# fabsig/GPBoost

Hardware: NVIDIA H100
Metric: gp_loglik_evals_per_sec (higher is better)
Workload: dtype f64

## Files before the change

### gpboost_b200/csrc/dev/dev_api.cu

```cuda
#include "../../../include/gpboost_b200_dev.h"

#include <cuda_runtime.h>

#include <algorithm>
#include <cmath>
#include <numeric>
#include <cstdio>
#include <cstring>
#include <string>
#include <vector>

#include "knn.cuh"
#include "vecchia_factor.cuh"
#include "vecchia_big.cuh"
#include "vecchia_nll2.cuh"

namespace {

thread_local std::string g_last_error;

int fail(const std::string& msg) {
  g_last_error = msg;
  return -1;
}

#define CUDA_TRY(expr)                                                                              \
  do {                                                                                              \
    cudaError_t err__ = (expr);                                                                     \
    if (err__ != cudaSuccess) {                                                                     \
      return fail(std::string("CUDA error at " __FILE__ ":") + std::to_string(__LINE__) + ": " +    \
                  cudaGetErrorString(err__));                                                       \
    }                                                                                               \
  } while (0)


__global__ void gather_perm_kernel(const double* __restrict__ src, const int32_t* __restrict__ perm,
                                   double* __restrict__ dst, int64_t n) {
  for (int64_t i = (int64_t)blockIdx.x * blockDim.x + threadIdx.x; i < n; i += (int64_t)gridDim.x * blockDim.x)
    dst[i] = src[perm[i]];
}

__global__ void reduce_partials_kernel(const double* __restrict__ partials, int64_t nrows, double* __restrict__ out) {
  __shared__ double sh[256];
  for (int k = 0; k < gpb::kNumAcc; ++k) {
    double s = 0.;
    for (int64_t r = threadIdx.x; r < nrows; r += blockDim.x) s += partials[r * gpb::kNumAcc + k];
    sh[threadIdx.x] = s;
    __syncthreads();
    for (int o = blockDim.x / 2; o > 0; o >>= 1) {
      if (threadIdx.x < o) sh[threadIdx.x] += sh[threadIdx.x + o];
      __syncthreads();
    }
    if (threadIdx.x == 0) out[k] = sh[0];
    __syncthreads();
  }
}

__global__ void bt_apply_kernel(const double* __restrict__ A, const double* __restrict__ u,
                                const int32_t* __restrict__ colptr, const int32_t* __restrict__ csc_pos,
                                const int32_t* __restrict__ perm, double* __restrict__ out_orig, int64_t n, int m,
                                int64_t row_begin, int64_t row_end, double scale) {
  const int lane = threadIdx.x & 31;
  const int64_t warp = ((int64_t)blockIdx.x * blockDim.x + threadIdx.x) >> 5;
  const int64_t nwarps = ((int64_t)gridDim.x * blockDim.x) >> 5;
  for (int64_t j = warp; j < n; j += nwarps) {
    const int32_t b = colptr[j], e = colptr[j + 1];
    double s = 0.;
    for (int32_t p = b + lane; p < e; p += 32) {
      const int32_t pos = csc_pos[p];
      s -= A[pos] * u[pos / m];
    }
    s = gpb::warp_sum(s);
    if (lane == 0) {
      if (j >= row_begin && j < row_end) s += u[j];
      out_orig[perm[j]] = s * scale;
    }
  }
}

__global__ void fill_kernel(double* p, int64_t n, double v) {
  for (int64_t i = (int64_t)blockIdx.x * blockDim.x + threadIdx.x; i < n; i += (int64_t)gridDim.x * blockDim.x) p[i] = v;
}

__global__ void fp64_peak_kernel(double* out, int iters, double a, double b) {
  double x0 = threadIdx.x, x1 = x0 + 1., x2 = x0 + 2., x3 = x0 + 3., x4 = x0 + 4., x5 = x0 + 5., x6 = x0 + 6., x7 = x0 + 7.;
  for (int i = 0; i < iters; ++i) {
    x0 = fma(x0, a, b); x1 = fma(x1, a, b); x2 = fma(x2, a, b); x3 = fma(x3, a, b);
    x4 = fma(x4, a, b); x5 = fma(x5, a, b); x6 = fma(x6, a, b); x7 = fma(x7, a, b);
  }
  if (x0 + x1 + x2 + x3 + x4 + x5 + x6 + x7 == 12345.678) out[0] = x0;
}

using FactorKernel = void (*)(const gpb::FactorArgs);

template <int COV, int MODE, int DIM>
FactorKernel pick_cap(int m) {
  if (m <= 10) return gpb::vecchia_factor_kernel<COV, MODE, DIM, 10>;
  if (m <= 20) return gpb::vecchia_factor_kernel<COV, MODE, DIM, 20>;
// ... 124 lines not shown
      const int32_t j = h->nn_host[(size_t)i * m + k];
      if (j >= 0) ++colptr[j + 1];
    }
  for (int64_t j = 0; j < n; ++j) colptr[j + 1] += colptr[j];
  std::vector<int32_t> pos((size_t)colptr[n]);
  std::vector<int32_t> fill(colptr.begin(), colptr.end() - 1);
  for (int64_t i = h->row_begin; i < h->row_end; ++i)
    for (int k = 0; k < m; ++k) {
      const int32_t j = h->nn_host[(size_t)i * m + k];
      if (j >= 0) pos[fill[j]++] = (int32_t)(i * m + k);
    }
  CUDA_TRY(cudaMalloc(&h->colptr, sizeof(int32_t) * (n + 1)));
  CUDA_TRY(cudaMalloc(&h->csc_pos, sizeof(int32_t) * std::max<size_t>(pos.size(), 1)));
  CUDA_TRY(cudaMemcpy(h->colptr, colptr.data(), sizeof(int32_t) * (n + 1), cudaMemcpyHostToDevice));
  CUDA_TRY(cudaMemcpy(h->csc_pos, pos.data(), sizeof(int32_t) * pos.size(), cudaMemcpyHostToDevice));
  CUDA_TRY(cudaMalloc(&h->yaux, sizeof(double) * n));
  return 0;
}

int launch_eval(gpbdev_vecchia* h, int cov_type, double var, double range, int mode, bool latent = false) {
  if (cov_type < 0 || cov_type > 3) return fail("gpbdev_vecchia_eval: unknown covariance id");
  if (mode < 0 || mode > 3) return fail("gpbdev_vecchia_eval: unknown mode");
  if (!(var > 0.) || !(range > 0.)) return fail("gpbdev_vecchia_eval: covariance parameters must be positive");
  CUDA_TRY(cudaSetDevice(h->device));
  if (mode == gpb::MODE_STORE && !latent && h->factor_stored && h->stored_cov == cov_type && h->stored_latent == latent &&
      h->stored_var == var && h->stored_range == range && h->last_cov == cov_type && h->last_latent == latent && h->last_var == var &&
      h->last_range == range)
    return 0;
  if (mode == gpb::MODE_STORE || mode == gpb::MODE_STORE_GRAD) {
    if (ensure_store_buffers(h)) return -1;
  }
  h->last_cov = cov_type; h->last_latent = latent; h->last_var = var; h->last_range = range;
  if (mode == gpb::MODE_STORE || mode == gpb::MODE_STORE_GRAD) { h->stored_cov = cov_type; h->stored_latent = latent; h->stored_var = var; h->stored_range = range; }
  if (mode == gpb::MODE_STORE_GRAD && !h->dA) {
    CUDA_TRY(cudaMalloc(&h->dA, sizeof(double) * h->n * h->m));
    CUDA_TRY(cudaMalloc(&h->dD, sizeof(double) * h->n));
    CUDA_TRY(cudaMemsetAsync(h->dA, 0, sizeof(double) * h->n * h->m, h->stream));
    CUDA_TRY(cudaMemsetAsync(h->dD, 0, sizeof(double) * h->n, h->stream));
  }
  gpb::FactorArgs a;
  a.coords = h->coords; a.nn = h->nn; a.y = h->y;
  a.A = h->A; a.Dinv = h->Dinv; a.w = h->u;
  a.partials = h->partials;
  a.n = h->n; a.row_begin = h->row_begin; a.row_end = h->row_end;
  a.m = h->m; a.d = h->d; a.var = var; a.range = range;
  a.diag_nb = latent ? var * (1. + 1e-10) : var + 1.;
  a.diag_obs = latent ? var : var + 1.;
  if (mode == gpb::MODE_STORE_GRAD) {
    CUDA_TRY(cudaMemcpyToSymbolAsync(gpb::g_factor_dA, &h->dA, sizeof(double*), 0, cudaMemcpyHostToDevice, h->stream));
    CUDA_TRY(cudaMemcpyToSymbolAsync(gpb::g_factor_dD, &h->dD, sizeof(double*), 0, cudaMemcpyHostToDevice, h->stream));
  }
  if (latent && mode == gpb::MODE_GRAD) return fail("gpbdev_vecchia_eval: the gradient pass assumes a Gaussian likelihood");
  auto finish = [&](int64_t rows) -> int {
    CUDA_TRY(cudaGetLastError());
    reduce_partials_kernel<<<1, 256, 0, h->stream>>>(h->partials, rows, h->sums);
    CUDA_TRY(cudaGetLastError());
    h->launches += 2;
    if (h->allreduce && !latent) {
      if (h->allreduce(h->allreduce_ctx, h->sums, gpb::kNumAcc, (void*)h->stream)) return fail("gpbdev_vecchia_eval: device all-reduce failed");
    }
    if (mode == gpb::MODE_STORE || mode == gpb::MODE_STORE_GRAD) h->factor_stored = true;
    return 0;
  };
  if (h->m > gpb::kMaxNeighbors) {
    if (mode == gpb::MODE_STORE_GRAD) return fail("gpbdev_vecchia_eval: the factor derivative (non-Gaussian likelihoods) supports num_neighbors <= 30");
    gpb::BigArgs b;
    b.coords = h->coords; b.y = h->y; b.nn = h->nn; b.qcoords = nullptr;
    b.A = h->A; b.Dinv = h->Dinv; b.w = h->u; b.pred_mean = nullptr; b.pred_var = nullptr; b.partials = h->partials;
    b.row_begin = h->row_begin; b.row_end = h->row_end; b.m = h->m; b.d = h->d;
    b.var = var; b.range = range; b.diag_nb = a.diag_nb; b.diag_obs = a.diag_obs;
    const int bmode = mode == gpb::MODE_NLL ? gpb::BIG_NLL : (mode == gpb::MODE_STORE ? gpb::BIG_STORE : gpb::BIG_GRAD);
    const int warps = bmode == gpb::BIG_GRAD ? 2 : 4;
    BigKernel bk = pick_big_kernel(cov_type, bmode);
    const size_t bsmem = gpb::big_smem_bytes(bmode, warps, h->d);
    CUDA_TRY(cudaFuncSetAttribute(bk, cudaFuncAttributeMaxDynamicSharedMemorySize, (int)bsmem));
    int grid = std::min(h->num_sms, (int)((h->grid_cap * gpb::kWarpsPerBlock) / warps));
    grid = std::max(grid, 1);
    bk<<<grid, warps * 32, bsmem, h->stream>>>(b);
    return finish((int64_t)grid * warps);
  }
  if ((mode == gpb::MODE_NLL || mode == gpb::MODE_STORE || (mode == gpb::MODE_GRAD && !latent)) && h->d == 2 && h->m > 20) {
    FactorKernel k2 = nullptr;
#define GPB_PICK2(COVID)                                                                                                              \
    k2 = mode == gpb::MODE_NLL ? gpb::vecchia_nll2_kernel<COVID, gpb::MODE_NLL>                                                      \
         : (mode == gpb::MODE_STORE ? gpb::vecchia_nll2_kernel<COVID, gpb::MODE_STORE> : gpb::vecchia_nll2_kernel<COVID, gpb::MODE_GRAD>)
    switch (cov_type) {
      case gpb::COV_EXPONENTIAL: GPB_PICK2(gpb::COV_EXPONENTIAL); break;
      case gpb::COV_MATERN15: GPB_PICK2(gpb::COV_MATERN15); break;
      case gpb::COV_MATERN25: GPB_PICK2(gpb::COV_MATERN25); break;
      default: GPB_PICK2(gpb::COV_GAUSSIAN); break;
    }
#undef GPB_PICK2
    const size_t smem2 = sizeof(double) * gpb::kWarpsPerBlock * 2 * (gpb::kNll2Half + 64);
    CUDA_TRY(cudaFuncSetAttribute(k2, cudaFuncAttributeMaxDynamicSharedMemorySize, (int)smem2));
    CUDA_TRY(cudaFuncSetAttribute(k2, cudaFuncAttributePreferredSharedMemoryCarveout, cudaSharedmemCarveoutMaxShared));
    int per_sm2 = 0;
    CUDA_TRY(cudaOccupancyMaxActiveBlocksPerMultiprocessor(&per_sm2, k2, gpb::kWarpsPerBlock * 32, smem2));
    int grid2 = std::max(per_sm2, 1) * h->num_sms;
    grid2 = std::max(1, std::min(grid2, h->grid_cap / 2));
    k2<<<grid2, gpb::kWarpsPerBlock * 32, smem2, h->stream>>>(a);
    if (finish((int64_t)grid2 * gpb::kWarpsPerBlock * 2)) return -1;
    if (mode == gpb::MODE_GRAD && a.A != nullptr) {
      h->factor_stored = true;
      h->stored_cov = cov_type; h->stored_latent = false; h->stored_var = var; h->stored_range = range;
    }
    return 0;
  }
  FactorKernel k = pick_kernel(cov_type, mode, h->d, h->m);
  if (!k) return fail("gpbdev_vecchia_eval: no one-observation factor kernel for this mode at d = 2, num_neighbors > 20");
  const size_t smem = sizeof(double) * gpb::kWarpsPerBlock * (32 * gpb::kLd + 32 * h->d + 64);
  CUDA_TRY(cudaFuncSetAttribute(k, cudaFuncAttributeMaxDynamicSharedMemorySize, (int)smem));
  CUDA_TRY(cudaFuncSetAttribute(k, cudaFuncAttributePreferredSharedMemoryCarveout, cudaSharedmemCarveoutMaxShared));
  int per_sm = 0;
  CUDA_TRY(cudaOccupancyMaxActiveBlocksPerMultiprocessor(&per_sm, k, gpb::kWarpsPerBlock * 32, smem));
  int grid = std::max(per_sm, 1) * h->num_sms;
  if (grid > h->grid_cap) grid = h->grid_cap;
  k<<<grid, gpb::kWarpsPerBlock * 32, smem, h->stream>>>(a);
  return finish((int64_t)grid * gpb::kWarpsPerBlock);
}

}

extern "C" {

const char* gpbdev_last_error(void) { return g_last_error.c_str(); }

int gpbdev_vecchia_set_allreduce(gpbdev_vecchia_t h, gpbdev_allreduce_fn fn, void* ctx) {
  if (!h) return fail("gpbdev_vecchia_set_allreduce: null argument");
  h->allreduce = fn;
  h->allreduce_ctx = ctx;
  return 0;
}

int gpbdev_device_count(void) {
  int c = 0;
  if (cudaGetDeviceCount(&c) != cudaSuccess) { cudaGetLastError(); return 0; }
  return c;
}

int gpbdev_vecchia_create(gpbdev_vecchia_t* out, int device, int64_t n, int d, int m, const double* coords_ordered,
                          const int32_t* perm, const int32_t* nn, int64_t row_begin, int64_t row_end) {
  if (!out || !coords_ordered || !perm) return fail("gpbdev_vecchia_create: null argument");
  if (n <= 0 || d <= 0 || d > 16) return fail("gpbdev_vecchia_create: need n > 0 and 1 <= dim <= 16");
  if (m < 1 || m > gpb::kBigMaxNeighbors)
    return fail("gpbdev_vecchia_create: num_neighbors must be in [1, " + std::to_string(gpb::kBigMaxNeighbors) +
                "] for the CUDA Vecchia engine");
  if ((int64_t)n * m >= (int64_t)2147483647) return fail("gpbdev_vecchia_create: n * num_neighbors exceeds int32 positions");
  if (row_begin < 0 || row_end > n || row_begin > row_end) return fail("gpbdev_vecchia_create: bad row shard");
  if (nn) {
    std::vector<int64_t> seen((size_t)n, -1);
    for (int64_t i = 0; i < n; ++i)
      for (int k = 0; k < m; ++k) {
        const int32_t j = nn[i * m + k];
        if (j == -1) continue;
        if (j < -1 || j >= i)
          return fail("gpbdev_vecchia_create: neighbour " + std::to_string(j) + " of row " + std::to_string(i) +
                      " is neither -1 nor an earlier row");
        if (seen[(size_t)j] == i)
          return fail("gpbdev_vecchia_create: neighbour " + std::to_string(j) + " appears twice in row " + std::to_string(i));
        seen[(size_t)j] = i;
      }
  }
  if (gpbdev_device_count() <= device)
    return fail("gpbdev_vecchia_create: no CUDA device " + std::to_string(device) + " — the CUDA engine has no CPU fallback");
  CUDA_TRY(cudaSetDevice(device));
  gpbdev_vecchia* h = new gpbdev_vecchia();
  h->device = device; h->n = n; h->d = d; h->m = m; h->row_begin = row_begin; h->row_end = row_end;
  cudaDeviceProp prop;
  CUDA_TRY(cudaGetDeviceProperties(&prop, device));
  h->num_sms = prop.multiProcessorCount;
  CUDA_TRY(cudaStreamCreateWithFlags(&h->stream, cudaStreamNonBlocking));
  CUDA_TRY(cudaEventCreate(&h->ev0));
  CUDA_TRY(cudaEventCreate(&h->ev1));
  CUDA_TRY(cudaMalloc(&h->coords, sizeof(double) * n * d));
  CUDA_TRY(cudaMalloc(&h->nn, sizeof(int32_t) * n * m));
  CUDA_TRY(cudaMalloc(&h->perm, sizeof(int32_t) * n));
// ... 263 lines not shown
  CUDA_TRY(cudaStreamSynchronize(h->stream));
  CUDA_TRY(cudaMemcpy(A_host, h->A, sizeof(double) * h->n * h->m, cudaMemcpyDeviceToHost));
  CUDA_TRY(cudaMemcpy(Dinv_host, h->Dinv, sizeof(double) * h->n, cudaMemcpyDeviceToHost));
  CUDA_TRY(cudaMemcpy(dA_host, h->dA, sizeof(double) * h->n * h->m, cudaMemcpyDeviceToHost));
  CUDA_TRY(cudaMemcpy(dD_host, h->dD, sizeof(double) * h->n, cudaMemcpyDeviceToHost));
  return 0;
}

int gpbdev_vecchia_get_factor(gpbdev_vecchia_t h, double* A_host, double* Dinv_host) {
  if (!h || !A_host || !Dinv_host) return fail("gpbdev_vecchia_get_factor: null argument");
  if (!h->factor_stored) return fail("gpbdev_vecchia_get_factor: call gpbdev_vecchia_eval(mode=STORE) first");
  CUDA_TRY(cudaSetDevice(h->device));
  CUDA_TRY(cudaStreamSynchronize(h->stream));
  CUDA_TRY(cudaMemcpy(A_host, h->A, sizeof(double) * h->n * h->m, cudaMemcpyDeviceToHost));
  CUDA_TRY(cudaMemcpy(Dinv_host, h->Dinv, sizeof(double) * h->n, cudaMemcpyDeviceToHost));
  return 0;
}

int gpbdev_vecchia_timer_start(gpbdev_vecchia_t h) {
  if (!h) return fail("null handle");
  CUDA_TRY(cudaSetDevice(h->device));
  CUDA_TRY(cudaEventRecord(h->ev0, h->stream));
  return 0;
}
int gpbdev_vecchia_timer_stop(gpbdev_vecchia_t h, float* ms) {
  if (!h || !ms) return fail("null argument");
  CUDA_TRY(cudaSetDevice(h->device));
  CUDA_TRY(cudaEventRecord(h->ev1, h->stream));
  CUDA_TRY(cudaEventSynchronize(h->ev1));
  CUDA_TRY(cudaEventElapsedTime(ms, h->ev0, h->ev1));
  return 0;
}
int gpbdev_vecchia_sync(gpbdev_vecchia_t h) {
  if (!h) return fail("null handle");
  CUDA_TRY(cudaSetDevice(h->device));
  CUDA_TRY(cudaStreamSynchronize(h->stream));
  return 0;
}
int64_t gpbdev_vecchia_launch_count(gpbdev_vecchia_t h) { return h ? h->launches : 0; }
int gpbdev_vecchia_knn_replayed(gpbdev_vecchia_t h) { return h ? h->knn_replayed : 0; }

int gpbdev_knn_search(int device, const double* coords_host, int64_t n, int d, int m, int64_t q_begin, int64_t end_search_at,
                      int32_t* nn_host, int64_t* info_out) {
  if (!coords_host || !nn_host || !info_out) return fail("gpbdev_knn_search: null argument");
  if (d < 1) return fail("gpbdev_knn_search: need dim >= 1");
  if (m < 1 || m > gpb::kBigMaxNeighbors)
    return fail("gpbdev_knn_search: num_neighbors must be in [1, " + std::to_string(gpb::kBigMaxNeighbors) + "]");
  if (n < 1 || n >= (int64_t)2147483647) return fail("gpbdev_knn_search: need 1 <= n < 2^31");
  if (q_begin < 0 || q_begin >= n) return fail("gpbdev_knn_search: q_begin must be in [0, n)");
  if (end_search_at != (q_begin == 0 ? n - 2 : q_begin - 1))
    return fail("gpbdev_knn_search: end_search_at must be n - 2 for model queries (q_begin = 0) and q_begin - 1 for prediction");
  m = (int)std::min<int64_t>(m, end_search_at + 1);
  if (m < 1) return fail("gpbdev_knn_search: model queries need n >= 2");
  const int64_t nq = n - q_begin;
  if (nq * m >= (int64_t)2147483647) return fail("gpbdev_knn_search: n * num_neighbors exceeds int32 positions");
  if (gpbdev_device_count() <= device) return fail("gpbdev_knn_search: no CUDA device " + std::to_string(device));
  CUDA_TRY(cudaSetDevice(device));
  cudaDeviceProp prop;
  CUDA_TRY(cudaGetDeviceProperties(&prop, device));
  cudaStream_t stream = nullptr;
  double* coords_dev = nullptr;
  int32_t* nn_dev = nullptr;
  CUDA_TRY(cudaStreamCreateWithFlags(&stream, cudaStreamNonBlocking));
  auto release = [&]() { cudaFree(coords_dev); cudaFree(nn_dev); cudaStreamDestroy(stream); };
  cudaError_t e = cudaMalloc(&coords_dev, sizeof(double) * n * d);
  if (e == cudaSuccess) e = cudaMalloc(&nn_dev, sizeof(int32_t) * nq * m);
  if (e == cudaSuccess) e = cudaMemcpy(coords_dev, coords_host, sizeof(double) * n * d, cudaMemcpyHostToDevice);
  if (e != cudaSuccess) { release(); return fail(std::string("gpbdev_knn_search: ") + cudaGetErrorString(e)); }
  std::string err;
  gpb::KnnInfo info;
  if (gpb::knn_vecchia_search(coords_dev, coords_host, n, d, m, nn_dev, stream, prop.multiProcessorCount, &info, &err, q_begin,
                              end_search_at) < 0) {
    release();
    return fail("gpbdev_knn_search: " + err);
  }
  e = cudaMemcpy(nn_host, nn_dev, sizeof(int32_t) * nq * m, cudaMemcpyDeviceToHost);
  release();
  if (e != cudaSuccess) return fail(std::string("gpbdev_knn_search: ") + cudaGetErrorString(e));
  const int64_t vals[7] = {info.replayed, info.launches, info.brute_end, info.ncell, info.g[0], info.g[1], info.g[2]};
  std::memcpy(info_out, vals, sizeof(vals));
  return 0;
}

int gpbdev_fp64_peak(int device, double* tflops) {
  if (!tflops) return fail("null argument");
  CUDA_TRY(cudaSetDevice(device));
  cudaDeviceProp prop;
  CUDA_TRY(cudaGetDeviceProperties(&prop, device));
  double* out = nullptr;
  CUDA_TRY(cudaMalloc(&out, 8));
  cudaEvent_t e0, e1;
  CUDA_TRY(cudaEventCreate(&e0));
  CUDA_TRY(cudaEventCreate(&e1));
  const int blocks = prop.multiProcessorCount * 8, threads = 256, iters = 1 << 14;
  fp64_peak_kernel<<<blocks, threads>>>(out, 1 << 10, 1.0000001, 1e-9);
  double best = 0.;
  for (int rep = 0; rep < 5; ++rep) {
    CUDA_TRY(cudaEventRecord(e0));
    fp64_peak_kernel<<<blocks, threads>>>(out, iters, 1.0000001, 1e-9);
    CUDA_TRY(cudaEventRecord(e1));
    CUDA_TRY(cudaEventSynchronize(e1));
    float ms = 0.f;
    CUDA_TRY(cudaEventElapsedTime(&ms, e0, e1));
    const double flops = 2.0 * 8 * (double)iters * blocks * threads;
    best = std::max(best, flops / (ms * 1e-3) / 1e12);
  }
  cudaEventDestroy(e0); cudaEventDestroy(e1); cudaFree(out);
  *tflops = best;
  return 0;
}

int gpbdev_vecchia_flush_l2(gpbdev_vecchia_t h) {
  if (!h) return fail("null handle");
  CUDA_TRY(cudaSetDevice(h->device));
  if (!h->flush) {
    h->flush_n = (int64_t)(256 << 20) / sizeof(double);
    CUDA_TRY(cudaMalloc(&h->flush, sizeof(double) * h->flush_n));
  }
  fill_kernel<<<h->num_sms * 8, 256, 0, h->stream>>>(h->flush, h->flush_n, 1.0);
  CUDA_TRY(cudaGetLastError());
  return 0;
}

}

#include "newton.cuh"
#include "covariates.cuh"
#include "laplace.cuh"
#include "fisher.cuh"
```

### include/gpboost_b200_dev.h

```cpp
#ifndef GPBOOST_B200_DEV_H_
#define GPBOOST_B200_DEV_H_
#include <stdint.h>
#ifdef __cplusplus
extern "C" {
#endif

#define GPBDEV_EXPORT __attribute__((visibility("default")))

enum { GPBDEV_COV_EXPONENTIAL = 0, GPBDEV_COV_MATERN15 = 1, GPBDEV_COV_MATERN25 = 2, GPBDEV_COV_GAUSSIAN = 3 };
enum { GPBDEV_MODE_NLL = 0, GPBDEV_MODE_STORE = 1, GPBDEV_MODE_GRAD = 2 };
enum {
  GPBDEV_SUM_QUAD = 0,
  GPBDEV_SUM_LOGDET = 1,
  GPBDEV_SUM_NBAD = 2,
  GPBDEV_SUM_UKU0 = 3, GPBDEV_SUM_UKU1 = 4,
  GPBDEV_SUM_UDU0 = 5, GPBDEV_SUM_UDU1 = 6,
  GPBDEV_SUM_TR0 = 7, GPBDEV_SUM_TR1 = 8,
  GPBDEV_NUM_SUMS = 9
};

typedef struct gpbdev_vecchia* gpbdev_vecchia_t;

GPBDEV_EXPORT const char* gpbdev_last_error(void);
GPBDEV_EXPORT int gpbdev_device_count(void);

GPBDEV_EXPORT int gpbdev_vecchia_create(gpbdev_vecchia_t* out, int device, int64_t n, int d, int m,
                                        const double* coords_ordered, const int32_t* perm,
                                        const int32_t* nn, int64_t row_begin, int64_t row_end);
GPBDEV_EXPORT int gpbdev_vecchia_free(gpbdev_vecchia_t h);

GPBDEV_EXPORT int gpbdev_vecchia_get_nn(gpbdev_vecchia_t h, int32_t* nn_host);

GPBDEV_EXPORT int gpbdev_vecchia_set_y(gpbdev_vecchia_t h, const double* y_host);
GPBDEV_EXPORT int gpbdev_vecchia_set_y_device(gpbdev_vecchia_t h, const double* y_dev);

GPBDEV_EXPORT int gpbdev_vecchia_eval(gpbdev_vecchia_t h, int cov_type, double var, double range, int mode,
                                      double* out);
GPBDEV_EXPORT int gpbdev_vecchia_eval_async(gpbdev_vecchia_t h, int cov_type, double var, double range, int mode);
GPBDEV_EXPORT int gpbdev_vecchia_last_sums(gpbdev_vecchia_t h, double* out);

GPBDEV_EXPORT int gpbdev_vecchia_yaux(gpbdev_vecchia_t h, double* yaux_host);
GPBDEV_EXPORT int gpbdev_vecchia_yaux_device(gpbdev_vecchia_t h, double* out_dev, double scale);
GPBDEV_EXPORT int gpbdev_vecchia_laplace_time_ops(gpbdev_vecchia_t h, int t, int reps, float* out_ms);
GPBDEV_EXPORT int gpbdev_vecchia_predict(gpbdev_vecchia_t h, int cov_type, double var, double range, const double* coords_pred_host,
                                         int64_t np, int num_neighbors_pred, double* mean_out_host, double* var_out_host);
typedef struct gpbdev_vecchia_predset* gpbdev_vecchia_predset_t;
GPBDEV_EXPORT int gpbdev_vecchia_predset_create(gpbdev_vecchia_t h, const double* coords_pred_host, int64_t np, int num_neighbors_pred,
                                                gpbdev_vecchia_predset_t* out);
GPBDEV_EXPORT int gpbdev_vecchia_predset_eval(gpbdev_vecchia_predset_t ps, int cov_type, double var, double range, const double** mean_dev,
                                              const double** var_dev);
GPBDEV_EXPORT int gpbdev_vecchia_predset_free(gpbdev_vecchia_predset_t ps);
GPBDEV_EXPORT int gpbdev_vecchia_newton_system(gpbdev_vecchia_t h, const int32_t* leaf_of_row_dev, int num_leaves, const double* grad_dev,
                                               double* M_host, double* rhs_host);
GPBDEV_EXPORT int gpbdev_vecchia_set_covariates(gpbdev_vecchia_t h, const double* X_colmajor_host, int p);
GPBDEV_EXPORT int gpbdev_vecchia_gls_gram(gpbdev_vecchia_t h, double* G_host, double* r_host);
GPBDEV_EXPORT int gpbdev_vecchia_gls_residual(gpbdev_vecchia_t h, const double* beta_host, double* out3);
GPBDEV_EXPORT int gpbdev_vecchia_latent_factor_grad(gpbdev_vecchia_t h, int cov_type, double var, double range, double* A_host,
                                                    double* Dinv_host, double* dA_host, double* dD_host);
GPBDEV_EXPORT int gpbdev_vecchia_fisher_info(gpbdev_vecchia_t h, int cov_type, double sigma2, double var, double range,
                                             const double* probes_colmajor, int t, double* FI9);
GPBDEV_EXPORT int gpbdev_vecchia_get_factor(gpbdev_vecchia_t h, double* A_host, double* Dinv_host);

GPBDEV_EXPORT int gpbdev_vecchia_timer_start(gpbdev_vecchia_t h);
GPBDEV_EXPORT int gpbdev_vecchia_timer_stop(gpbdev_vecchia_t h, float* ms);
GPBDEV_EXPORT int gpbdev_vecchia_sync(gpbdev_vecchia_t h);
GPBDEV_EXPORT int64_t gpbdev_vecchia_launch_count(gpbdev_vecchia_t h);
GPBDEV_EXPORT int gpbdev_vecchia_knn_replayed(gpbdev_vecchia_t h);
GPBDEV_EXPORT int gpbdev_knn_search(int device, const double* coords_host, int64_t n, int d, int m, int64_t q_begin,
                                    int64_t end_search_at, int32_t* nn_host, int64_t* info_out);
typedef int (*gpbdev_allreduce_fn)(void* ctx, double* dev_buf, int64_t count, void* stream);
GPBDEV_EXPORT int gpbdev_vecchia_set_allreduce(gpbdev_vecchia_t h, gpbdev_allreduce_fn fn, void* ctx);
GPBDEV_EXPORT int gpbdev_fp64_peak(int device, double* tflops);
GPBDEV_EXPORT int gpbdev_vecchia_flush_l2(gpbdev_vecchia_t h);

enum { GPBDEV_LIK_BERNOULLI_LOGIT = 0, GPBDEV_LIK_POISSON = 1 };
GPBDEV_EXPORT int gpbdev_vecchia_laplace_set_likelihood(gpbdev_vecchia_t h, int likelihood, double log_norm_const);
GPBDEV_EXPORT int gpbdev_laplace_rows(int device, int likelihood, int64_t n, const double* y_host, const double* mode_host,
                                      const double* fe_host, const double* Dinv_host, double* out_host);
GPBDEV_EXPORT int gpbdev_vecchia_laplace_set_probes(gpbdev_vecchia_t h, const double* probes_colmajor, int t);
GPBDEV_EXPORT int gpbdev_vecchia_laplace_eval(gpbdev_vecchia_t h, int cov_type, double var, double range,
                                              const double* fixed_effects_host, const double* cfg, double* out);
GPBDEV_EXPORT int gpbdev_vecchia_laplace_get_mode(gpbdev_vecchia_t h, double* mode_host);
GPBDEV_EXPORT int gpbdev_vecchia_laplace_keep_solutions(gpbdev_vecchia_t h, int keep);
GPBDEV_EXPORT int gpbdev_vecchia_laplace_grad(gpbdev_vecchia_t h, int cov_type, double var, double range, const double* cfg, double* out);
GPBDEV_EXPORT int gpbdev_vecchia_laplace_set_collective(gpbdev_vecchia_t h, void (*allreduce_sum)(double*, int), int t_total);
GPBDEV_EXPORT int gpbdev_vecchia_laplace_apply(gpbdev_vecchia_t h, int cov_type, double var, double range, int op, int t,
                                               const double* W_host, const double* X_host, const double* X2_host, double* out_host,
                                               double* dots_host);

typedef struct gpbdev_dense* gpbdev_dense_t;
GPBDEV_EXPORT const char* gpbdev_dense_last_error(void);
GPBDEV_EXPORT int gpbdev_dense_create(gpbdev_dense_t* out, int device, int n, int d, const double* coords_rowmajor);
GPBDEV_EXPORT int gpbdev_dense_free(gpbdev_dense_t h);
GPBDEV_EXPORT int gpbdev_dense_set_y(gpbdev_dense_t h, const double* y_host);
GPBDEV_EXPORT int gpbdev_dense_eval(gpbdev_dense_t h, int cov_type, double var, double range, double* out3);
GPBDEV_EXPORT int gpbdev_dense_yaux(gpbdev_dense_t h, double scale, double* yaux_host);
GPBDEV_EXPORT int gpbdev_dense_grad(gpbdev_dense_t h, double* out4);
GPBDEV_EXPORT int gpbdev_dense_get_factor(gpbdev_dense_t h, double* L_host, double* z_host);
GPBDEV_EXPORT int gpbdev_dense_get_psi_inv(gpbdev_dense_t h, double* P_host);
GPBDEV_EXPORT int64_t gpbdev_dense_launch_count(gpbdev_dense_t h);

typedef struct gpbdev_grouped* gpbdev_grouped_t;
GPBDEV_EXPORT const char* gpbdev_grouped_last_error(void);
GPBDEV_EXPORT int gpbdev_grouped_create(gpbdev_grouped_t* out, int device, int64_t n, const int32_t* group_index, int num_groups);
GPBDEV_EXPORT int gpbdev_grouped_free(gpbdev_grouped_t h);
GPBDEV_EXPORT int gpbdev_grouped_set_y(gpbdev_grouped_t h, const double* y_host);
GPBDEV_EXPORT int gpbdev_grouped_eval(gpbdev_grouped_t h, double var_ratio, double* out5);
GPBDEV_EXPORT int gpbdev_grouped_yaux(gpbdev_grouped_t h, double var_ratio, double scale, double* yaux_host);
GPBDEV_EXPORT int gpbdev_grouped_set_y_device(gpbdev_grouped_t h, const double* y_dev);
GPBDEV_EXPORT int gpbdev_grouped_yaux_device(gpbdev_grouped_t h, double var_ratio, double scale, double* out_dev);
GPBDEV_EXPORT int64_t gpbdev_grouped_launch_count(gpbdev_grouped_t h);

typedef struct gpbdev_grouped_multi* gpbdev_grouped_multi_t;
GPBDEV_EXPORT int gpbdev_grouped_multi_create(gpbdev_grouped_multi_t* out, int device, int64_t n, int K, const int32_t* level_index,
                                              const int* num_levels);
GPBDEV_EXPORT int gpbdev_grouped_multi_free(gpbdev_grouped_multi_t h);
GPBDEV_EXPORT int gpbdev_grouped_multi_info(gpbdev_grouped_multi_t h, int64_t* out2);
GPBDEV_EXPORT int gpbdev_grouped_multi_set_y(gpbdev_grouped_multi_t h, const double* y_host);
GPBDEV_EXPORT int gpbdev_grouped_multi_set_y_device(gpbdev_grouped_multi_t h, const double* y_dev);
GPBDEV_EXPORT int gpbdev_grouped_multi_set_probes(gpbdev_grouped_multi_t h, const double* probes, int t);
GPBDEV_EXPORT int gpbdev_grouped_multi_eval(gpbdev_grouped_multi_t h, const double* v, const double* cfg, double* out5);
GPBDEV_EXPORT int gpbdev_grouped_multi_grad(gpbdev_grouped_multi_t h, double sigma2, double* grad);
GPBDEV_EXPORT int gpbdev_grouped_multi_yaux(gpbdev_grouped_multi_t h, const double* v, const double* cfg, double scale, double* out,
                                            int out_is_device, int* its);
GPBDEV_EXPORT int gpbdev_grouped_multi_apply(gpbdev_grouped_multi_t h, const double* v, int which, const double* X, int t, double* Y);
GPBDEV_EXPORT int gpbdev_grouped_multi_time_ops(gpbdev_grouped_multi_t h, int reps, float* out_ms);
GPBDEV_EXPORT int64_t gpbdev_grouped_multi_launch_count(gpbdev_grouped_multi_t h);

typedef struct gpbdev_tree* gpbdev_tree_t;
typedef struct {
  int num_leaves;
  int min_data_in_leaf;
  double min_sum_hessian_in_leaf;
  double lambda_l2;
  double min_gain_to_split;
  int max_depth;
} gpbdev_tree_config;

GPBDEV_EXPORT const char* gpbdev_tree_last_error(void);
GPBDEV_EXPORT int gpbdev_tree_create(gpbdev_tree_t* out, int device, int64_t n, int F, const uint8_t* bins_feature_major,
                                     const int32_t* num_bin, const gpbdev_tree_config* cfg);
GPBDEV_EXPORT int gpbdev_tree_create_on_device_bins(gpbdev_tree_t* out, int device, int64_t n, int F, int Fpad, const uint8_t* bins_dev,
                                                    const int32_t* num_bin, const gpbdev_tree_config* cfg);
GPBDEV_EXPORT int gpbdev_tree_free(gpbdev_tree_t h);

GPBDEV_EXPORT const char* gpbdev_bin_last_error(void);
GPBDEV_EXPORT int gpbdev_bin_matrix(int device, const void* data_host, int data_type, int64_t nrow, int ncol, int is_row_major, int F,
                                    const int32_t* real_feature, const int32_t* num_bin, const double* upper_bounds,
                                    int upper_bounds_stride, int Fpad, uint8_t** bins_dev_out);
GPBDEV_EXPORT int gpbdev_bin_free(int device, uint8_t* bins_dev);
GPBDEV_EXPORT int gpbdev_bin_download(int device, const uint8_t* bins_dev, int64_t nrow, int Fpad, uint8_t* out_host);
GPBDEV_EXPORT int gpbdev_tree_train(gpbdev_tree_t h, const double* grad, int grad_on_device, double hess_const, int* num_leaves,
                                    int* split_feature, int* threshold_bin, int* left_child, int* right_child, float* split_gain,
                                    double* leaf_value, int* leaf_count);
GPBDEV_EXPORT int gpbdev_tree_add_score(gpbdev_tree_t h, const double* leaf_values, int num_leaves, double* score_dev,
// ... 41 lines not shown
```

Baseline: 323.8.

## Add FP64 tensor-core blocked Cholesky kernel for Vecchia NLL evaluation

After: 346.3, median of 6. 1.07x the previous value.

```diff
diff --git a/gpboost_b200/csrc/dev/dev_api.cu b/gpboost_b200/csrc/dev/dev_api.cu
--- a/gpboost_b200/csrc/dev/dev_api.cu
+++ b/gpboost_b200/csrc/dev/dev_api.cu
@@ -14,6 +14,7 @@
 #include "vecchia_factor.cuh"
 #include "vecchia_big.cuh"
 #include "vecchia_nll2.cuh"
+#include "vecchia_nll_mma.cuh"
 
 namespace {
 
@@ -304,7 +305,7 @@
   if ((mode == gpb::MODE_NLL || mode == gpb::MODE_STORE || (mode == gpb::MODE_GRAD && !latent)) && h->d == 2 && h->m > 20) {
     FactorKernel k2 = nullptr;
 #define GPB_PICK2(COVID)                                                                                                              \
-    k2 = mode == gpb::MODE_NLL ? gpb::vecchia_nll2_kernel<COVID, gpb::MODE_NLL>                                                      \
+    k2 = mode == gpb::MODE_NLL ? gpb::vecchia_nll_mma_kernel<COVID>                                                                  \
          : (mode == gpb::MODE_STORE ? gpb::vecchia_nll2_kernel<COVID, gpb::MODE_STORE> : gpb::vecchia_nll2_kernel<COVID, gpb::MODE_GRAD>)
     switch (cov_type) {
       case gpb::COV_EXPONENTIAL: GPB_PICK2(gpb::COV_EXPONENTIAL); break;
@@ -313,7 +314,8 @@
       default: GPB_PICK2(gpb::COV_GAUSSIAN); break;
     }
 #undef GPB_PICK2
-    const size_t smem2 = sizeof(double) * gpb::kWarpsPerBlock * 2 * (gpb::kNll2Half + 64);
+    const size_t smem2 = mode == gpb::MODE_NLL ? gpb::kWarpsPerBlock * gpb::kMmaSmemPerWarp
+                                               : sizeof(double) * gpb::kWarpsPerBlock * 2 * (gpb::kNll2Half + 64);
     CUDA_TRY(cudaFuncSetAttribute(k2, cudaFuncAttributeMaxDynamicSharedMemorySize, (int)smem2));
     CUDA_TRY(cudaFuncSetAttribute(k2, cudaFuncAttributePreferredSharedMemoryCarveout, cudaSharedmemCarveoutMaxShared));
     int per_sm2 = 0;
@@ -743,6 +745,20 @@
   return 0;
 }
 
+int gpbdev_dmma_m8n8k4(const double* a, const double* b, const double* c, double* d) {
+  if (!a || !b || !c || !d) return fail("gpbdev_dmma_m8n8k4: null argument");
+  double* buf = nullptr;
+  CUDA_TRY(cudaMalloc(&buf, sizeof(double) * (32 + 32 + 64 + 64)));
+  CUDA_TRY(cudaMemcpy(buf, a, sizeof(double) * 32, cudaMemcpyHostToDevice));
+  CUDA_TRY(cudaMemcpy(buf + 32, b, sizeof(double) * 32, cudaMemcpyHostToDevice));
+  CUDA_TRY(cudaMemcpy(buf + 64, c, sizeof(double) * 64, cudaMemcpyHostToDevice));
+  gpb::dmma_m8n8k4_check_kernel<<<1, 32>>>(buf, buf + 32, buf + 64, buf + 128);
+  CUDA_TRY(cudaGetLastError());
+  CUDA_TRY(cudaMemcpy(d, buf + 128, sizeof(double) * 64, cudaMemcpyDeviceToHost));
+  CUDA_TRY(cudaFree(buf));
+  return 0;
+}
+
 int gpbdev_fp64_peak(int device, double* tflops) {
   if (!tflops) return fail("null argument");
   CUDA_TRY(cudaSetDevice(device));
diff --git a/gpboost_b200/csrc/dev/vecchia_nll_mma.cuh b/gpboost_b200/csrc/dev/vecchia_nll_mma.cuh
--- /dev/null
+++ b/gpboost_b200/csrc/dev/vecchia_nll_mma.cuh
@@ -0,0 +1,247 @@
+#pragma once
+#include "vecchia_nll2.cuh"
+
+namespace gpb {
+
+constexpr int kMmaHalf = 16 * 32 + 16 * 16 + 2;
+constexpr size_t kMmaSmemPerWarp = sizeof(double) * 2 * (kMmaHalf + 64);
+
+__device__ __forceinline__ int mma_at(int r, int c) {
+  const int h = (c & 2) | ((c ^ (c >> 2)) & 1);
+  return (c < 16 ? c * 32 : 240 + c * 16) + (r ^ (h << 2));
+}
+
+__device__ __forceinline__ void dmma_m8n8k4(double& d0, double& d1, double a, double b) {
+  asm("mma.sync.aligned.m8n8k4.row.col.f64.f64.f64.f64 {%0, %1}, {%2}, {%3}, {%0, %1};" : "+d"(d0), "+d"(d1) : "d"(a), "d"(b));
+}
+
+__global__ void dmma_m8n8k4_check_kernel(const double* A, const double* B, const double* C, double* D) {
+  const int lane = threadIdx.x & 31, g = lane >> 2, t = lane & 3;
+  double d0 = C[g * 8 + 2 * t], d1 = C[g * 8 + 2 * t + 1];
+  dmma_m8n8k4(d0, d1, A[g * 4 + t], B[t * 8 + g]);
+  D[g * 8 + 2 * t] = d0;
+  D[g * 8 + 2 * t + 1] = d1;
+}
+
+template <int PN>
+__device__ __forceinline__ void nll_mma_panel(double* W, double* S, int hl, int hbase, int g, int t, double& Di) {
+  constexpr int MT = 30;
+  constexpr int K0 = 8 * PN;
+  constexpr int KE = PN == 3 ? MT + 1 : K0 + 8;
+  constexpr bool LO = K0 < 16;
+  double pl[8], ph[8];
+#pragma unroll
+  for (int j = 0; j < KE - K0; ++j) {
+    pl[j] = LO ? S[mma_at(hl, K0 + j)] : 0.;
+    ph[j] = S[mma_at(hl + 16, K0 + j)];
+  }
+  double dg_lo = LO ? S[mma_at(hl, hl)] : 0., dg_hi = S[mma_at(hl + 16, hl + 16)];
+  double lk_lo, lk_hi;
+  {
+    const double d0 = LO ? __shfl_sync(0xffffffffu, dg_lo, hbase + K0) : __shfl_sync(0xffffffffu, dg_hi, hbase + K0 - 16);
+    const double r0 = rsqrt_fast(d0);
+    lk_lo = pl[0] * r0; lk_hi = ph[0] * r0;
+    if (LO) S[mma_at(hl, K0)] = lk_lo;
+    S[mma_at(hl + 16, K0)] = lk_hi;
+  }
+  __syncwarp();
+#pragma unroll
+  for (int j = 0; j + 1 < KE - K0; ++j) {
+    const int k = K0 + j;
+    dg_lo = fma(-lk_lo, lk_lo, dg_lo);
+    dg_hi = fma(-lk_hi, lk_hi, dg_hi);
+    const double dn = (k + 1 < 16) ? __shfl_sync(0xffffffffu, dg_lo, hbase + k + 1) : __shfl_sync(0xffffffffu, dg_hi, hbase + k + 1 - 16);
+    {
+      const double m1 = S[mma_at(k + 1, k)];
+      ph[j + 1] -= lk_hi * m1;
+      if (LO) pl[j + 1] -= lk_lo * m1;
+    }
+    if (k + 1 == MT) Di = dn;
+    const double rn = rsqrt_fast(dn);
+    const double lk1_lo = LO ? pl[j + 1] * rn : 0.;
+    const double lk1_hi = ph[j + 1] * rn;
+    if (((k + 2) & 1) && k + 2 < KE) {
+      const double l1 = S[mma_at(k + 2, k)];
+      ph[j + 2] -= lk_hi * l1;
+      if (LO) pl[j + 2] -= lk_lo * l1;
+    }
+#pragma unroll
+    for (int c = (k + 3) & ~1; c < KE; c += 2) {
+      const double2 l2 = *reinterpret_cast<const double2*>(&S[mma_at(c, k)]);
+      ph[c - K0] -= lk_hi * l2.x;
+      if (c + 1 < KE) ph[c + 1 - K0] -= lk_hi * l2.y;
+      if (LO) {
+        pl[c - K0] -= lk_lo * l2.x;
+        if (c + 1 < KE) pl[c + 1 - K0] -= lk_lo * l2.y;
+      }
+    }
+    if (LO) S[mma_at(hl, k + 1)] = lk1_lo;
+    S[mma_at(hl + 16, k + 1)] = lk1_hi;
+    __syncwarp();
+    lk_lo = lk1_lo; lk_hi = lk1_hi;
+  }
+  if (PN < 3) {
+#pragma unroll
+    for (int h2 = 0; h2 < 2; ++h2) {
+      double* T = W + h2 * kMmaHalf;
+      double f[3][2];
+#pragma unroll
+      for (int X = PN + 1; X < 4; ++X)
+#pragma unroll
+        for (int kk = 0; kk < 2; ++kk) f[X - PN - 1][kk] = T[mma_at(8 * X + g, K0 + 4 * kk + t)];
+#pragma unroll
+      for (int I = PN + 1; I < 4; ++I)
+#pragma unroll
+        for (int J = PN + 1; J <= I; ++J) {
+          const int a0 = mma_at(8 * I + g, 8 * J + 2 * t), a1 = mma_at(8 * I + g, 8 * J + 2 * t + 1);
+          double d0 = T[a0], d1 = T[a1];
+          dmma_m8n8k4(d0, d1, -f[I - PN - 1][0], f[J - PN - 1][0]);
+          dmma_m8n8k4(d0, d1, -f[I - PN - 1][1], f[J - PN - 1][1]);
+          T[a0] = d0; T[a1] = d1;
+        }
+    }
+    __syncwarp();
+  }
+}
+
+#ifndef GPB_NLL_MMA_BLOCKS
+#define GPB_NLL_MMA_BLOCKS 4
+#endif
+
+template <int COV>
+__global__ void __launch_bounds__(kWarpsPerBlock * 32, GPB_NLL_MMA_BLOCKS) vecchia_nll_mma_kernel(const FactorArgs p) {
+  constexpr int MT = 30, P = 31;
+  extern __shared__ __align__(16) double smem_raw[];
+  const int lane = threadIdx.x & 31, hl = lane & 15, hh = lane >> 4, wib = threadIdx.x >> 5;
+  const int hbase = lane & 16;
+  double* W = smem_raw + (size_t)wib * (2 * (kMmaHalf + 64));
+  double* S = W + (size_t)hh * kMmaHalf;
+  double* pts = W + 2 * kMmaHalf + (size_t)hh * 64;
+  const int64_t gwarp = (int64_t)blockIdx.x * kWarpsPerBlock + wib, nwarps = (int64_t)gridDim.x * kWarpsPerBlock;
+  const int m = p.m;
+  const double var = p.var;
+  const double sc = COV == COV_GAUSSIAN ? sqrt(p.range) : p.range;
+  const double logvar = log(var);
+  const double tab = kExp2Tab32[lane];
+  double acc0 = 0., acc1 = 0., acc2 = 0.;
+
+  auto slot_src = [&](int64_t ii, int s) -> int {
+    const int qq = ii < m ? (int)ii : m;
+    if (s < qq) return p.nn[ii * m + s];
+    return s == MT ? (int)ii : -1;
+  };
+  auto row_of = [&](int64_t it) -> int64_t { return p.row_begin + 2 * it + hh; };
+  int64_t it = gwarp;
+  int64_t i = row_of(it);
+  bool active = i < p.row_end;
+  int s_lo = -1, s_hi = -1, sn_lo = -1, sn_hi = -1;
+  double2 c_lo = make_double2(0., 0.), c_hi = c_lo;
+  double y_lo = 0., y_hi = 0.;
+  auto fetch_idx = [&](int64_t ii, bool act, int& a_lo, int& a_hi) {
+    a_lo = -1; a_hi = -1;
+    if (act) {
+      a_lo = slot_src(ii, hl);
+      a_hi = hl + 16 <= MT ? slot_src(ii, hl + 16) : -1;
+    }
+  };
+  auto fetch_data = [&]() {
+    y_lo = 0.; y_hi = 0.;
+    if (s_lo >= 0) { y_lo = p.y[s_lo]; c_lo = *reinterpret_cast<const double2*>(p.coords + (int64_t)s_lo * 2); }
+    if (s_hi >= 0) { y_hi = p.y[s_hi]; c_hi = *reinterpret_cast<const double2*>(p.coords + (int64_t)s_hi * 2); }
+  };
+  fetch_idx(i, active, s_lo, s_hi);
+  fetch_data();
+  fetch_idx(row_of(it + nwarps), row_of(it + nwarps) < p.row_end, sn_lo, sn_hi);
+
+  for (; __any_sync(0xffffffffu, active); ) {
+    int lane_it = lane;
+    asm volatile("" : "+r"(lane_it));
+    const int hl = lane_it & 15, g = lane_it >> 2, t = lane_it & 3;
+    const bool real_lo = s_lo >= 0, real_hi = s_hi >= 0;
+    const double2 my_lo = make_double2(c_lo.x * sc, c_lo.y * sc), my_hi = make_double2(c_hi.x * sc, c_hi.y * sc);
+    const double yl = y_lo, yh = y_hi;
+    if (real_lo) *reinterpret_cast<double2*>(pts + hl * 2) = my_lo;
+    if (real_hi) *reinterpret_cast<double2*>(pts + (hl + 16) * 2) = my_hi;
+    const unsigned blo = __ballot_sync(0xffffffffu, real_lo), bhi = __ballot_sync(0xffffffffu, real_hi);
+    const unsigned real_mask = ((blo >> hbase) & 0xffffu) | (((bhi >> hbase) & 0xffffu) << 16);
+    const bool full = (__all_sync(0xffffffffu, real_mask == (1u << P) - 1u || !active)) != 0;
+    const bool was_active = active;
+    const int64_t it_n = it + nwarps;
+    const int64_t i_n = row_of(it_n);
+    const bool active_n = i_n < p.row_end;
+    __syncwarp();
+
+    constexpr int NR = 2 * (MT / 2);
+    constexpr int G = GPB_NLL2_GROUP;
+    static_assert(NR % G == 0, "group size must divide the number of rounds");
+#pragma unroll
+    for (int r0 = 0; r0 < NR; r0 += G) {
+      double val[G];
+#pragma unroll
+      for (int j = 0; j < G; ++j) {
+        const int r = r0 + j;
+        const int tt = (r >> 1) + 1;
+        const bool odd = (r & 1) != 0;
+        const int pi = hl + (odd ? 16 : 0);
+        int o = pi + tt;
+        if (o >= P) o -= P;
+        if (pi >= P) o = 0;
+        const double2 po = *reinterpret_cast<const double2*>(pts + o * 2);
+        const double2 me = odd ? my_hi : my_lo;
+        const double dx = me.x - po.x, dy = me.y - po.y;
+        const double d2s = fma(dy, dy, fma(dx, dx, 1e-300));
+        double gd = 0.;
+        val[j] = cov_eval_scaled<COV, false>(d2s, var, logvar, tab, gd);
+      }
+#pragma unroll
+      for (int j = 0; j < G; ++j) {
+        const int r = r0 + j;
+        const int tt = (r >> 1) + 1;
+        const bool odd = (r & 1) != 0;
+        const int pi = hl + (odd ? 16 : 0);
+        const bool valid = pi < P;
+        int o = pi + tt;
+        if (o >= P) o -= P;
+        if (!valid) o = 0;
+        const bool keep = ((full ? 1u : 0u) | ((odd ? (unsigned)real_hi : (unsigned)real_lo) & (real_mask >> o) & 1u)) != 0u;
+        const double v = keep ? val[j] : 0.;
+        S[valid ? mma_at(max(pi, o), min(pi, o)) : mma_at(hl + 16, 31)] = v;
+      }
+    }
+    s_lo = sn_lo; s_hi = sn_hi;
+    fetch_data();
+    {
+      const int64_t i_n2 = row_of(it_n + nwarps);
+      fetch_idx(i_n2, i_n2 < p.row_end, sn_lo, sn_hi);
+    }
+    S[mma_at(hl, hl)] = real_lo ? p.diag_nb : 1.;
+    S[mma_at(MT + 1, hl)] = yl;
+    if (hl + 16 <= MT) {
+      S[mma_at(hl + 16, hl + 16)] = real_hi ? (hl + 16 == MT ? p.diag_obs : p.diag_nb) : 1.;
+      S[mma_at(MT + 1, hl + 16)] = yh;
+    }
+    __syncwarp();
+
+    double Di = 0.;
+    nll_mma_panel<0>(W, S, hl, hbase, g, t, Di);
+    nll_mma_panel<1>(W, S, hl, hbase, g, t, Di);
+    nll_mma_panel<2>(W, S, hl, hbase, g, t, Di);
+    nll_mma_panel<3>(W, S, hl, hbase, g, t, Di);
+    const double r_over_sd = S[mma_at(MT + 1, MT)];
+    if (hl == 0 && was_active) {
+      acc0 += r_over_sd * r_over_sd;
+      acc1 += log(Di);
+      acc2 += !(Di > 0.) ? 1. : 0.;
+    }
+    __syncwarp();
+    it = it_n; i = i_n; active = active_n;
+  }
+  if (hl == 0) {
+    double* out = p.partials + (size_t)(gwarp * 2 + hh) * kNumAcc;
+    out[0] = acc0; out[1] = acc1; out[2] = acc2;
+#pragma unroll
+    for (int k = 3; k < kNumAcc; ++k) out[k] = 0.;
+  }
+}
+
+}
diff --git a/include/gpboost_b200_dev.h b/include/gpboost_b200_dev.h
--- a/include/gpboost_b200_dev.h
+++ b/include/gpboost_b200_dev.h
@@ -71,6 +71,7 @@
 typedef int (*gpbdev_allreduce_fn)(void* ctx, double* dev_buf, int64_t count, void* stream);
 GPBDEV_EXPORT int gpbdev_vecchia_set_allreduce(gpbdev_vecchia_t h, gpbdev_allreduce_fn fn, void* ctx);
 GPBDEV_EXPORT int gpbdev_fp64_peak(int device, double* tflops);
+GPBDEV_EXPORT int gpbdev_dmma_m8n8k4(const double* a, const double* b, const double* c, double* d);
 GPBDEV_EXPORT int gpbdev_vecchia_flush_l2(gpbdev_vecchia_t h);
 
 enum { GPBDEV_LIK_BERNOULLI_LOGIT = 0, GPBDEV_LIK_POISSON = 1 };
```
